# nlesc-dirac/sagecal

Measured on NVIDIA H100. Metric: baseline_visibilities_per_sec_predict_jacobian, higher is better.
Workload: dtype f64

## Files before the change

sagecal_b200/csrc/internal.cuh:

```cuda
#pragma once
#include <cuda_runtime.h>
#include <stdint.h>
#include <stdio.h>
#include <stdlib.h>

#define DB_CHECK(call)                                                                          \
  do {                                                                                          \
    cudaError_t err__ = (call);                                                                 \
    if (err__ != cudaSuccess) {                                                                 \
      fprintf(stderr, "dirac_b200: CUDA error %s at %s:%d: %s\n", cudaGetErrorName(err__),      \
              __FILE__, __LINE__, cudaGetErrorString(err__));                                   \
      exit(1);          \
    }                                                                                           \
  } while (0)


#define TILE_P 8
#define TILE_Q 32
#define TILE_THREADS (TILE_P * TILE_Q)

struct TileDesc {
  short pb, qb;
};

// ... 86 lines not shown
}
__host__ __device__ __forceinline__ void cdot2c_acc(double2 &acc, double2 a0, double2 b0, double2 a1,
                                           double2 b1) {
  acc.x = fma(a0.x, b0.x, acc.x);
  acc.x = fma(a0.y, b0.y, acc.x);
  acc.x = fma(a1.x, b1.x, acc.x);
  acc.x = fma(a1.y, b1.y, acc.x);
  acc.y = fma(a0.y, b0.x, acc.y);
  acc.y = fma(-a0.x, b0.y, acc.y);
  acc.y = fma(a1.y, b1.x, acc.y);
  acc.y = fma(-a1.x, b1.y, acc.y);
}
__host__ __device__ __forceinline__ void mat_ab(const double2 *a, const double2 *b, double2 *c) {
  c[0] = cdot2(a[0], b[0], a[1], b[2]);
  c[1] = cdot2(a[0], b[1], a[1], b[3]);
  c[2] = cdot2(a[2], b[0], a[3], b[2]);
  c[3] = cdot2(a[2], b[1], a[3], b[3]);
}
__host__ __device__ __forceinline__ void mat_abh(const double2 *a, const double2 *b, double2 *c) {
  c[0] = cdot2c(a[0], b[0], a[1], b[1]);
  c[1] = cdot2c(a[0], b[2], a[1], b[3]);
  c[2] = cdot2c(a[2], b[0], a[3], b[1]);
  c[3] = cdot2c(a[2], b[2], a[3], b[3]);
}
__host__ __device__ __forceinline__ void mat_abh_acc(const double2 *a, const double2 *b, double2 *c) {
  cdot2c_acc(c[0], a[0], b[0], a[1], b[1]);
  cdot2c_acc(c[1], a[0], b[2], a[1], b[3]);
  cdot2c_acc(c[2], a[2], b[0], a[3], b[1]);
  cdot2c_acc(c[3], a[2], b[2], a[3], b[3]);
}
__host__ __device__ __forceinline__ void mat_ahb(const double2 *a, const double2 *b, double2 *c) {
  c[0] = cadd(cmulcl(a[0], b[0]), cmulcl(a[2], b[2]));
  c[1] = cadd(cmulcl(a[0], b[1]), cmulcl(a[2], b[3]));
  c[2] = cadd(cmulcl(a[1], b[0]), cmulcl(a[3], b[2]));
  c[3] = cadd(cmulcl(a[1], b[1]), cmulcl(a[3], b[3]));
}

__device__ __forceinline__ double2 ld_stream(const double2 *p) {
  double2 v;
  asm volatile("ld.global.nc.L1::no_allocate.v2.f64 {%0,%1}, [%2];" : "=d"(v.x), "=d"(v.y) : "l"(p));
  return v;
}
__device__ __forceinline__ void st_stream(double2 *p, double2 v) {
  asm volatile("st.global.L1::no_allocate.v2.f64 [%0], {%1,%2};" ::"l"(p), "d"(v.x), "d"(v.y)
               : "memory");
}

__device__ __forceinline__ double warp_sum(double v) {
#pragma unroll
  for (int o = 16; o > 0; o >>= 1) v += __shfl_xor_sync(0xffffffffu, v, o);
  return v;
}

__device__ __forceinline__ void load_jones(const double *pblk, int sta, double2 *J) {
  const double2 *s = reinterpret_cast<const double2 *>(pblk + 8 * (long long)sta);
  J[0] = __ldg(s + 0);
  J[1] = __ldg(s + 1);
  J[2] = __ldg(s + 2);
  J[3] = __ldg(s + 3);
}

__device__ __forceinline__ int row_chunk(long long r, long long R, int nchunk) {
  return nchunk == 1 ? 0 : (int)(r / ((R + nchunk - 1) / nchunk));
}

struct GradArgs {
  const double2 *coh;
  const double2 *res;
  const unsigned char *flag;
  const double *pp;
  const ClusterDesc *clus;
  const int *chunk_poff;
  const TileDesc *tiles;
  double *g;
  long long R;
  int N, Nbase, tilesz, M;
  int robust;
  double nu;
  double scale;
  int tb0;
  long long w_lo, w_hi;
};

struct ClusterPassArgs {
  const double2 *coh_k;
  const double2 *in;
  const unsigned char *flag;
  const double *pblk;
  const TileDesc *tiles;
  double2 *out;
  double *jte;
  double *partials;
  double *cost;
  unsigned int *counter;
  long long R;
  int N, Nbase;
  int t_begin, t_end, tslice;
  int mode;
  int write_out;
  double beta;
  const double *pblk_old;
  int form_hidden;
  const short2 *blpq;
  double *jte_part;
  unsigned int *gcounter;
  const double2 *wt;
};

struct WeightedJtjArgs {
  const double2 *coh_k;
  const double2 *wt;
  const unsigned char *flag;
  const double *pblk;
  const TileDesc *tiles;
  double *JTJ;
  double *HP, *HQ;
  long long R;
  int N, Nbase;
  int t_begin, t_end, tslice;
};

// ... 110 lines not shown
```

sagecal_b200/csrc/kernels_line.cu:

```cuda
#include "internal.cuh"

__device__ __forceinline__ void grid_reduce_sum_l(double v, double *partials, double *out,
                                                  unsigned int *counter) {
  __shared__ double wsum[32];
  __shared__ bool is_last;
  v = warp_sum(v);
  const int lane = threadIdx.x & 31, w = threadIdx.x >> 5;
  if (lane == 0) wsum[w] = v;
  __syncthreads();
  const unsigned int nblocks = gridDim.x * gridDim.y;
  const unsigned int bid = blockIdx.x + gridDim.x * blockIdx.y;
  if (threadIdx.x == 0) {
    double s = 0.0;
    const int nw = (blockDim.x + 31) >> 5;
    for (int i = 0; i < nw; i++) s += wsum[i];
    partials[bid] = s;
    __threadfence();
    is_last = (atomicAdd(counter, 1u) == nblocks - 1);
  }
  __syncthreads();
  if (is_last) {
    double s = 0.0;
    for (unsigned int i = threadIdx.x; i < nblocks; i += blockDim.x)
      s += ((volatile double *)partials)[i];
// ... 62 lines not shown
    out[threadIdx.x] = s;
    if (threadIdx.x == 0) *counter = 0;
  }
}

__global__ void __launch_bounds__(256)
k_line_poly(const double2 *__restrict__ E0, const double2 *__restrict__ E1,
            const double2 *__restrict__ E2, long long n4, double *partials, double *out,
            unsigned int *counter) {
  double c[5] = {0.0, 0.0, 0.0, 0.0, 0.0};
  for (long long i = (long long)blockIdx.x * blockDim.x + threadIdx.x; i < n4;
       i += (long long)gridDim.x * blockDim.x) {
    const double2 e0 = E0[i], e1 = E1[i], e2 = E2[i];
    c[0] = fma(e0.x, e0.x, fma(e0.y, e0.y, c[0]));
    c[1] = fma(e0.x, e1.x, fma(e0.y, e1.y, c[1]));
    c[2] = fma(e1.x, e1.x, fma(e1.y, e1.y, c[2]));
    c[2] = fma(-2.0 * e0.x, e2.x, fma(-2.0 * e0.y, e2.y, c[2]));
    c[3] = fma(e1.x, e2.x, fma(e1.y, e2.y, c[3]));
    c[4] = fma(e2.x, e2.x, fma(e2.y, e2.y, c[4]));
  }
  poly_grid_reduce(c, partials, out, counter);
}

__global__ void __launch_bounds__(256)
k_line_poly_finish(const double *__restrict__ part, unsigned nparts, double *partials, double *out,
                   unsigned int *counter) {
  double c[5] = {0.0, 0.0, 0.0, 0.0, 0.0};
  for (unsigned i = blockIdx.x * blockDim.x + threadIdx.x; i < nparts; i += gridDim.x * blockDim.x)
#pragma unroll
    for (int j = 0; j < 5; j++) c[j] += part[(size_t)j * nparts + i];
  poly_grid_reduce(c, partials, out, counter);
}

__global__ void __launch_bounds__(256)
k_sumsq(const double2 *__restrict__ v, long long n4, double *partials, double *out,
        unsigned int *counter) {
  double s = 0.0;
  for (long long i = (long long)blockIdx.x * blockDim.x + threadIdx.x; i < n4;
       i += (long long)gridDim.x * blockDim.x) {
    const double2 e = v[i];
    s = fma(e.x, e.x, s);
    s = fma(e.y, e.y, s);
  }
  grid_reduce_sum_l(s, partials, out, counter);
}

__global__ void __launch_bounds__(256)
k_line_residual(const double2 *__restrict__ E0, const double2 *__restrict__ E1,
                const double2 *__restrict__ E2, double2 *__restrict__ res, long long n4,
                double alpha) {
  const double a2 = alpha * alpha;
  for (long long i = (long long)blockIdx.x * blockDim.x + threadIdx.x; i < n4;
       i += (long long)gridDim.x * blockDim.x) {
    const double2 e0 = E0[i], e1 = E1[i], e2 = E2[i];
    res[i] = make_double2((e0.x - alpha * e1.x) - a2 * e2.x, (e0.y - alpha * e1.y) - a2 * e2.y);
  }
}

__global__ void __launch_bounds__(256)
k_residual_cost(const double2 *__restrict__ x, const double2 *__restrict__ pm,
                double2 *__restrict__ out, long long n4, int out_mode, int cost_mode, double inv_nu,
                double *partials, double *cost, unsigned int *counter) {
  double s = 0.0;
  for (long long i = (long long)blockIdx.x * blockDim.x + threadIdx.x; i < n4;
       i += (long long)gridDim.x * blockDim.x) {
    const double2 xv = x[i], m = pm[i];
    const double2 e = make_double2(xv.x - m.x, xv.y - m.y);
    if (out_mode == 1) out[i] = e;
    if (out_mode == 2) out[i] = m;
    if (cost_mode == 1) {
      s = fma(e.x, e.x, s);
      s = fma(e.y, e.y, s);
    } else if (cost_mode == 2) {
      s += log(1.0 + e.x * e.x * inv_nu);
      s += log(1.0 + e.y * e.y * inv_nu);
    }
  }
  if (cost_mode) grid_reduce_sum_l(s, partials, cost, counter);
}

__global__ void __launch_bounds__(256)
k_axpby(const double2 *__restrict__ x, double2 *__restrict__ y, long long n4, double a, double b) {
  for (long long i = (long long)blockIdx.x * blockDim.x + threadIdx.x; i < n4;
       i += (long long)gridDim.x * blockDim.x) {
    const double2 xv = x[i], yv = y[i];
    y[i] = make_double2(a * xv.x + b * yv.x, a * xv.y + b * yv.y);
  }
}

__global__ void __launch_bounds__(256)
k_cluster_rowmap(const double2 *__restrict__ coh_k, const double2 *__restrict__ in,
                 const double2 *in2, double2 *out,
                 const unsigned char *__restrict__ flag, const double *__restrict__ pp,
                 const int *__restrict__ chunk_poff, int nchunk, const short2 *__restrict__ blpq,
                 long long R, int Nbase, int sign, double beta) {
  for (long long r = (long long)blockIdx.x * blockDim.x + threadIdx.x; r < R;
       r += (long long)gridDim.x * blockDim.x) {
    const short2 pq = blpq[r % Nbase];
    const int off = chunk_poff[row_chunk(r, R, nchunk)];
    double2 Jp[4], Jq[4], C[4], A[4], m[4];
    load_jones(pp + off, pq.x, Jp);
    load_jones(pp + off, pq.y, Jq);
#pragma unroll
    for (int c = 0; c < 4; c++) C[c] = coh_k[(long long)c * R + r];
    mat_ab(Jp, C, A);
    mat_abh(A, Jq, m);
    const bool fl = flag[r] != 0;
#pragma unroll
// ... 63 lines not shown
```

sagecal_b200/csrc/kernels_stream.cu:

```cuda
#include "internal.cuh"
#include "tma.cuh"

#define XP_ROWS 8
__global__ void k_coh_to_planar(const double2 *__restrict__ src, double2 *__restrict__ dst,
                                long long r0, int nr, int M, long long R) {
  __shared__ double2 tile[4][XP_ROWS][33];
  const int kx = blockIdx.x * 32 + threadIdx.x;
  const int ry = blockIdx.y * XP_ROWS + threadIdx.y;
  if (kx < M && ry < nr) {
    const double2 *s = src + ((long long)ry * M + kx) * 4;
#pragma unroll
    for (int c = 0; c < 4; c++) tile[c][threadIdx.y][threadIdx.x] = s[c];
  }
  __syncthreads();
  const int tid = threadIdx.y * 32 + threadIdx.x;
  const int rr = tid % XP_ROWS, kk = tid / XP_ROWS;
  const int k = blockIdx.x * 32 + kk;
  const int r = blockIdx.y * XP_ROWS + rr;
  if (k < M && r < nr) {
#pragma unroll
    for (int c = 0; c < 4; c++) dst[((long long)k * 4 + c) * R + r0 + r] = tile[c][rr][kk];
  }
}

// ... 92 lines not shown
template <int TB, int NST, bool WIN, bool BAND = false>
__device__ __forceinline__ void grad_tma_split_body(GradArgs a) {
  if (BAND) {
    a.coh += (long long)blockIdx.z * a.M * 4 * a.R;
    a.res += (long long)blockIdx.z * 4 * a.R;
  }
  extern __shared__ __align__(128) unsigned char smem_raw[];
  constexpr int STAGE_ELEMS = TB * 4 * 32;
  double (*sq)[8][TILE_Q] = reinterpret_cast<double (*)[8][TILE_Q]>(smem_raw);
  double2 *ring = reinterpret_cast<double2 *>(smem_raw + sizeof(double) * 2 * TILE_P * 8 * TILE_Q);
  unsigned long long *bars =
      reinterpret_cast<unsigned long long *>(ring + (size_t)TILE_P * NST * STAGE_ELEMS);
  const TileDesc td = a.tiles[blockIdx.x];
  const int h = threadIdx.x >> 8, w = (threadIdx.x >> 5) & 7, lane = threadIdx.x & 31;
  const int p = td.pb * TILE_P + w;
  const int q0 = td.qb * TILE_Q;
  const int q = q0 + lane;
  const bool valid = (q > p) && (q < a.N);
  const int t0 = (WIN ? a.tb0 + (int)blockIdx.y : (int)blockIdx.y) * TB;
  const int nrows = min(TB, a.tilesz - t0);
  const int qs = max(q0, p + 1);
  const int nv = max(0, min(q0 + TILE_Q, a.N) - qs);
  const long long b0 = nv > 0 ? baseline_index(p, qs, a.N) : 0;
  const int el = q - qs;
  const long long b = valid ? b0 + el : 0;
  double2 *my_stage = ring + (size_t)w * NST * STAGE_ELEMS;
  unsigned long long *my_bar = bars + w * NST;
  if (h == 0 && lane == 0) {
#pragma unroll
    for (int s = 0; s < NST; s++) mbar_init(&my_bar[s], 1);
    mbar_fence_init();
  }
  __syncthreads();
  auto issue = [&](int k, int s) {
    const unsigned row_bytes = (unsigned)nv * 16u;
    mbar_expect_tx(&my_bar[s], (unsigned)nrows * 4u * row_bytes);
    const double2 *ck = a.coh + (long long)k * 4 * a.R + (long long)t0 * a.Nbase + b0;
    double2 *dst = my_stage + (size_t)s * STAGE_ELEMS;
    for (int i = 0; i < nrows; i++)
#pragma unroll
      for (int c = 0; c < 4; c++)
        bulk_g2s(dst + (i * 4 + c) * 32, ck + (long long)c * a.R + (long long)i * a.Nbase, row_bytes,
                 &my_bar[s]);
  };
  const bool producer = (h == 0 && lane == 0 && nv > 0);
  if (producer) {
#pragma unroll
    for (int s = 0; s < NST - 1; s++)
      if (s < a.M) issue(s, s);
  }

  double2 Rm[TB][2];
  bool use[TB];
#pragma unroll
  for (int i = 0; i < TB; i++) {
    const int t = t0 + i;
    const long long row = (long long)(t < a.tilesz ? t : a.tilesz - 1) * a.Nbase + b;
    use[i] = valid && (t < a.tilesz) && (a.flag[row] == 0);
    if (WIN) use[i] = use[i] && row >= a.w_lo && row < a.w_hi;
#pragma unroll
    for (int j = 0; j < 2; j++) {
      double2 e = make_double2(0.0, 0.0);
      if (use[i]) {
        e = ld_stream(a.res + (long long)(2 * h + j) * a.R + row);
        if (a.robust) {
          e.x = e.x / (a.nu + e.x * e.x);
          e.y = e.y / (a.nu + e.y * e.y);
        }
      }
      Rm[i][j] = e;
    }
  }
  for (int k = 0; k < a.M; k++) {
    const int s = k % NST;
    if (producer && k + NST - 1 < a.M) issue(k + NST - 1, (k + NST - 1) % NST);
    const ClusterDesc cd = a.clus[k];
    const int tpc = (a.tilesz + cd.nchunk - 1) / cd.nchunk;
    if (nv > 0) mbar_wait(&my_bar[s], (unsigned)((k / NST) & 1));
    const double2 *st = my_stage + (size_t)s * STAGE_ELEMS;
    int i0 = 0;
    while (i0 < TB) {
      int chunk = 0, i1 = TB;
      double2 W[8];
#pragma unroll
      for (int z = 0; z < 8; z++) W[z] = make_double2(0.0, 0.0);
      if (cd.nchunk == 1) {
#pragma unroll
        for (int i = 0; i < TB; i++) {
          if (use[i]) {
            double2 C[4];
#pragma unroll
            for (int c = 0; c < 4; c++) C[c] = lds_v2(st + (i * 4 + c) * 32 + el);
#pragma unroll
            for (int j = 0; j < 2; j++)
#pragma unroll
              for (int lm = 0; lm < 4; lm++) cfmac(W[j * 4 + lm], Rm[i][j], C[lm]);
          }
        }
      } else {
        chunk = (t0 + i0 < a.tilesz ? t0 + i0 : a.tilesz - 1) / tpc;
        i1 = i0;
#pragma unroll
        for (int i = 0; i < TB; i++) {
          if (i >= i0 && i == i1) {
            const int t = t0 + i;
            const int ch = (t < a.tilesz ? t : a.tilesz - 1) / tpc;
            if (ch == chunk) {
              i1 = i + 1;
              if (use[i]) {
                double2 C[4];
#pragma unroll
                for (int c = 0; c < 4; c++) C[c] = lds_v2(st + (i * 4 + c) * 32 + el);
#pragma unroll
                for (int j = 0; j < 2; j++)
#pragma unroll
                  for (int lm = 0; lm < 4; lm++) cfmac(W[j * 4 + lm], Rm[i][j], C[lm]);
              }
// ... 506 lines not shown
      for (int i = tid; i < n8; i += 512) {
        double sacc = 0.0;
        for (unsigned c = 0; c < gridDim.y; c++) sacc += __ldcg(grp + (size_t)c * n8 + i);
        if (sacc != 0.0) atomicAdd(a.jte + i, sacc);
      }
      if (tid == 0) a.gcounter[blockIdx.x] = 0;
    }
  }
  grid_reduce_sum(cost, a.partials, a.cost, a.counter);
}


__global__ void __launch_bounds__(TILE_THREADS)
k_coh_gram(GramArgs a) {
  const TileDesc td = a.tiles[blockIdx.x];
  const int w = threadIdx.x >> 5, lane = threadIdx.x & 31;
  const int p = td.pb * TILE_P + w;
  const int q = td.qb * TILE_Q + lane;
  if (!((q > p) && (q < a.N))) return;
  const long long b = baseline_index(p, q, a.N);
  const double2 *ck = a.coh + (long long)(a.k0 + blockIdx.y) * 4 * a.R;
  double d[4] = {0.0, 0.0, 0.0, 0.0};
  double2 o[6];
#pragma unroll
  for (int z = 0; z < 6; z++) o[z] = make_double2(0.0, 0.0);
#pragma unroll 4
  for (int t = a.t_begin; t < a.t_end; t += a.t_step) {
    const long long row = (long long)t * a.Nbase + b;
    double2 C[4];
#pragma unroll
    for (int c = 0; c < 4; c++) C[c] = ld_stream(ck + (long long)c * a.R + row);
    if (a.flag[row] == 0) {
#pragma unroll
      for (int c = 0; c < 4; c++) {
        d[c] = fma(C[c].x, C[c].x, d[c]);
        d[c] = fma(C[c].y, C[c].y, d[c]);
      }
      cfmacl(o[0], C[0], C[1]);
      cfmacl(o[1], C[0], C[2]);
      cfmacl(o[2], C[0], C[3]);
      cfmacl(o[3], C[1], C[2]);
      cfmacl(o[4], C[1], C[3]);
      cfmacl(o[5], C[2], C[3]);
    }
  }
  double2 *Tb = reinterpret_cast<double2 *>(a.T + ((long long)blockIdx.y * a.Nbase + b) * 16);
  Tb[0] = make_double2(d[0], d[1]);
  Tb[1] = make_double2(d[2], d[3]);
#pragma unroll
  for (int z = 0; z < 6; z++) Tb[2 + z] = o[z];
}

void db_launch_grad_tma(const GradArgs *a, int ntile, cudaStream_t st) {
  constexpr int TB = 4, NST = 2;
  const size_t smem = sizeof(double) * 2 * TILE_P * 8 * TILE_Q +
                      (size_t)TILE_P * NST * TB * 4 * 32 * sizeof(double2) + TILE_P * NST * 8;
  static bool configured = false;
  if (!configured) {
    DB_CHECK(cudaFuncSetAttribute(k_grad_tma_split<TB, NST>,
                                  cudaFuncAttributeMaxDynamicSharedMemorySize, (int)smem));
    configured = true;
  }
  dim3 grid(ntile, (a->tilesz + TB - 1) / TB);
  k_grad_tma_split<TB, NST><<<grid, 2 * TILE_THREADS, smem, st>>>(*a);
}

void db_launch_grad_band_tma(const GradArgs *a, int ntile, int nchan, cudaStream_t st) {
  constexpr int TB = 4, NST = 2;
  const size_t smem = sizeof(double) * 2 * TILE_P * 8 * TILE_Q +
                      (size_t)TILE_P * NST * TB * 4 * 32 * sizeof(double2) + TILE_P * NST * 8;
  static bool configured = false;
  if (!configured) {
    DB_CHECK(cudaFuncSetAttribute(k_grad_tma_band<TB, NST>,
                                  cudaFuncAttributeMaxDynamicSharedMemorySize, (int)smem));
    configured = true;
  }
  dim3 grid(ntile, (a->tilesz + TB - 1) / TB, nchan);
  k_grad_tma_band<TB, NST><<<grid, 2 * TILE_THREADS, smem, st>>>(*a);
}

void db_launch_grad_window_tma(const GradArgs *a, int ntile, long long r_lo, long long r_hi,
                               cudaStream_t st) {
  constexpr int TB = 4, NST = 2;
  if (r_hi <= r_lo) return;
  const size_t smem = sizeof(double) * 2 * TILE_P * 8 * TILE_Q +
                      (size_t)TILE_P * NST * TB * 4 * 32 * sizeof(double2) + TILE_P * NST * 8;
  static bool configured = false;
  if (!configured) {
    DB_CHECK(cudaFuncSetAttribute(k_grad_tma_window<TB, NST>,
                                  cudaFuncAttributeMaxDynamicSharedMemorySize, (int)smem));
    configured = true;
  }
  const int t_lo = (int)(r_lo / a->Nbase), t_hi = (int)((r_hi + a->Nbase - 1) / a->Nbase);
  const int tb_lo = t_lo / TB, tb_hi = (t_hi + TB - 1) / TB;
  GradArgs b = *a;
  b.tb0 = tb_lo;
  b.w_lo = r_lo;
  b.w_hi = r_hi;
  dim3 grid(ntile, tb_hi - tb_lo);
  k_grad_tma_window<TB, NST><<<grid, 2 * TILE_THREADS, smem, st>>>(b);
}

static bool cluster_pass_lin_fits(int N, int Nbase) {
  return (size_t)5 * 8 * 256 * sizeof(double2) + sizeof(double) * ((8 * N + 1) & ~1) + 40 <=
             (size_t)200 * 1024 && (Nbase + 255) / 256 <= 1024;
}

// ... 79 lines not shown
```

sagecal_b200/csrc/lbfgs.cu:

```cuda
#include <float.h>
#include <math.h>
#include <string.h>
#include <vector>

#include "problem.h"

extern "C" {
int db_lbfgs_direction_max_pairs(void);
void db_launch_lbfgs_direction(double *pk, const double *gk, const double *s, const double *y,
                               const double *rho, int m, int npairs, int next, cudaStream_t st);
void db_launch_lbfgs_nrm2(const double *g, int m, double *out, cudaStream_t st);
void db_launch_lbfgs_step(const double *xk, const double *pk, const double *gk, double *xk1,
                          double *sk, double *yk, int m, double alpha, cudaStream_t st);
void db_launch_lbfgs_update(const double *gk, const double *sk, double *yk, const double *xk1,
                            double *xk, int m, double *rho_slot, double *out, cudaStream_t st);
void db_launch_line_eval(const double2 *E0, const double2 *E1, const double2 *E2, long long n4,
                         double alpha, int mode, double inv_nu, double *partials, double *out,
                         unsigned int *counter, cudaStream_t st);
void db_launch_line_residual(const double2 *E0, const double2 *E1, const double2 *E2, double2 *res,
                             long long n4, double alpha, cudaStream_t st);
void db_launch_line_poly(const double2 *E0, const double2 *E1, const double2 *E2, long long n4,
                         double *partials, double *out, unsigned int *counter, cudaStream_t st);
}

// ... 66 lines not shown
    }
    db_prof_end(d.stream);
    DB_CHECK(cudaEventRecord(ev_done, cs));
    DB_CHECK(cudaStreamWaitEvent(d.stream, ev_done, 0));
    db_launch_axpby(d.x, pr->E0, 4 * d.R, 1.0, -1.0, d.stream);
    db_count_launch(1);
  } else {
    db_prof_begin(7, (double)d.R * (64.0 * d.M + 65.0 + 192.0), d.stream);
    const unsigned nparts = db_launch_line_setup_tma(&s, d.stream);
    db_prof_end(d.stream);
    db_count_launch(1);
    if (fold_poly) {
      db_launch_line_poly_finish(pr->poly_part, nparts, pr->partials, d.scal + 16, d.counters,
                                 d.stream);
      db_count_launch(1);
    }
    if (pr->world > 1) {
      db_allreduce(pr, pr->E0, 3 * 8 * d.R);
      db_launch_axpby(d.x, pr->E0, 4 * d.R, 1.0, -1.0, d.stream);
      db_count_launch(1);
    }
  }
  if (want_poly) {
    if (!fold_poly) {
      db_launch_line_poly(pr->E0, pr->E1, pr->E2, 4 * d.R, pr->partials, d.scal + 16, d.counters,
                          d.stream);
      db_count_launch(1);
    }
    DB_CHECK(cudaMemcpyAsync(d.h_scal + 16, d.scal + 16, 5 * sizeof(double), cudaMemcpyDeviceToHost,
                             d.stream));
    db_stream_sync(d.stream);
    for (int j = 0; j < 5; j++) c->poly[j] = d.h_scal[16 + j];
  }
}

static double line_cost(LbfgsCtx *c, double alpha) {
  dirac_b200_problem *pr = c->pr;
  DevProblem &d = pr->d;
  if (!c->robust && !db_opt(DB_OPT_LINE_DIRECT)) {
    c->ncost++;
    const double *q = c->poly;
    return q[0] + alpha * (q[1] + alpha * (q[2] + alpha * (q[3] + alpha * q[4])));
  }
  db_launch_line_eval(pr->E0, pr->E1, pr->E2, 4 * d.R, alpha, c->robust ? 2 : 1,
                      c->robust ? 1.0 / c->nu : 0.0, pr->partials, d.scal, d.counters, d.stream);
  db_count_launch(1);
  c->ncost++;
  return db_read_scalar(pr, 0);
}

enum { RES_PREDICT, RES_LINE, RES_HELD };
static void grad_eval(LbfgsCtx *c, const double *p, double *g, int res_src, double alpha) {
  dirac_b200_problem *pr = c->pr;
  DevProblem &d = pr->d;
  if (res_src == RES_LINE) {
    db_launch_line_residual(pr->E0, pr->E1, pr->E2, pr->res, 4 * d.R, alpha, d.stream);
    db_count_launch(1);
  } else if (res_src == RES_PREDICT) {
    db_predict_dev(pr, p, pr->res, 1, 0, 0.0, 0);
  }
  db_grad_dev(pr, p, g, c->robust, c->nu);
  c->ngrad++;
}

static double cubic_interp(LbfgsCtx *c, double a, double b, double *xa, double step) {
  double f0, f1, f0d, f1d, p01, p02, z0, fz0, aa, cc;
  *xa = a;
  f0 = line_cost(c, *xa);
  *xa += step;
  p01 = line_cost(c, *xa);
  *xa += -2.0 * step;
  p02 = line_cost(c, *xa);
  f0d = (p01 - p02) / (2.0 * step);
  *xa += -a + step + b;
  f1 = line_cost(c, *xa);
  *xa += step;
  p01 = line_cost(c, *xa);
  *xa += -2.0 * step;
  p02 = line_cost(c, *xa);
  f1d = (p01 - p02) / (2.0 * step);

  aa = 3.0 * (f0 - f1) / (b - a) + (f1d - f0d);
  p01 = aa * aa - f0d * f1d;
  if (p01 > 0.0) {
    cc = sqrt(p01);
    z0 = b - (f1d + cc - aa) * (b - a) / (f1d - f0d + 2.0 * cc);
    aa = (a > b) ? a : b;
    cc = (a < b) ? a : b;
    if (z0 > aa || z0 < cc) {
      fz0 = f0 + f1;
    } else {
      *xa += -b + step + a + z0 * (b - a);
      fz0 = line_cost(c, *xa);
    }
    if (f0 < f1 && f0 < fz0) return a;
    if (f1 < fz0) return b;
    return z0;
  }
  return (f0 < f1) ? a : b;
}

static double linesearch_zoom(LbfgsCtx *c, double a, double b, double *xa, double phi_0,
                              double gphi_0, double sigma, double rho, double t1, double t2,
                              double t3, double step) {
  double alphaj = 0.0, phi_j, phi_aj, gphi_j, p01, p02, aj = a, bj = b, alphak = 1.0;
  int ci = 0, found_step = 0;
  (void)t1;
  while (ci < 10) {
    p01 = aj + t2 * (bj - aj);
    p02 = bj - t3 * (bj - aj);
    alphaj = cubic_interp(c, p01, p02, xa, step);
    *xa = alphaj;
    phi_j = line_cost(c, *xa);
    *xa += -alphaj + aj;
// ... 81 lines not shown
    ci++;
  }
  return alphak;
}

struct LbfgsTrace {
  double *alphak;
  long long *ncost;
  int *slot;
  double *gnorm;
  double *iterates;
  int niter;
};

static int lbfgs_run(dirac_b200_problem *pr, double *p, int m, int itmax, int M, int robust,
                      double nu, bool res_held, LbfgsTrace *tr) {
  DevProblem &d = pr->d;
  LbfgsCtx ctx;
  ctx.pr = pr;
  ctx.robust = robust;
  ctx.nu = nu;
  ctx.m = m;
  ctx.ncost = ctx.ngrad = 0;
  if (tr) tr->niter = 0;
  if (M < 1) M = 1;
  if (M > db_lbfgs_direction_max_pairs()) {
    fprintf(stderr, "dirac_b200: LBFGS memory size %d exceeds the %d pairs the two-loop recursion "
                    "can hold; the LBFGS stage is skipped\n", M, db_lbfgs_direction_max_pairs());
    return 0;
  }
  double *ws = (double *)db_malloc(sizeof(double) * ((size_t)m * (4 + 2 * (size_t)M) + M + 8));
  double *xk = ws, *xk1 = xk + m, *gk = xk1 + m, *pk = gk + m, *s = pk + m,
         *y = s + (size_t)m * M, *rho = y + (size_t)m * M;
  double *nrm_dev = d.scal + 24;
  double step, alphak;
  int ck, ci, cm;
  DB_CHECK(cudaMemcpyAsync(xk, p, sizeof(double) * m, cudaMemcpyHostToDevice, d.stream));
  grad_eval(&ctx, xk, gk, res_held ? RES_HELD : RES_PREDICT, 0.0);
  db_launch_lbfgs_nrm2(gk, m, nrm_dev, d.stream);
  db_count_launch(1);
  double gradnrm = sqrt(db_read_scalar(pr, 24));
  const double STOP = 1e-17;
  if (gradnrm < STOP) {
    ck = itmax;
    step = 0.0;
  } else {
    ck = 0;
    double t = 1e-3 / gradnrm;
    if (t > 1e-6) t = 1e-6;
    step = (t > 1e-9) ? t : 1e-9;
  }
  cm = 0;
  ci = 0;
  while (ck < itmax && isnormal(gradnrm) && gradnrm > STOP) {
    const long long ncost0 = ctx.ncost;
    db_launch_lbfgs_direction(pk, gk, s, y, rho, m, ck < M ? ck : M, ci, d.stream);
    db_count_launch(1);
    line_setup(&ctx, xk, pk);
    alphak = linesearch(&ctx, 10.0, 0.1, 0.01, 9, 0.1, 0.5, step);
    if (!isnormal(alphak) || fabs(alphak) < 1e-12) break;
    double *sk = s + (size_t)cm;
    double *yk = y + (size_t)cm;
    db_launch_lbfgs_step(xk, pk, gk, xk1, sk, yk, m, alphak, d.stream);
    grad_eval(&ctx, xk1, gk, RES_LINE, alphak);
    db_launch_lbfgs_update(gk, sk, yk, xk1, xk, m, rho + ci, nrm_dev, d.stream);
    db_count_launch(2);
    gradnrm = sqrt(db_read_scalar(pr, 24));
    if (tr) {
      tr->alphak[ck] = alphak;
      tr->ncost[ck] = ctx.ncost - ncost0;
      tr->slot[ck] = ci;
      tr->gnorm[ck] = gradnrm;
      DB_CHECK(cudaMemcpy(tr->iterates + (size_t)m * ck, xk, sizeof(double) * m,
                          cudaMemcpyDeviceToHost));
      tr->niter = ck + 1;
    }
    ck++;
    if (cm < (M - 1) * m) {
      cm += m;
      ci++;
    } else {
      cm = ci = 0;
    }
  }
  DB_CHECK(cudaMemcpyAsync(p, xk, sizeof(double) * m, cudaMemcpyDeviceToHost, d.stream));
  db_stream_sync(d.stream);
  db_free(ws);
  return (int)ctx.ngrad - 1;
}

int db_lbfgs_fit(dirac_b200_problem *pr, double *p, int m, int itmax, int M, int robust,
                 double nu, bool res_held) {
  return lbfgs_run(pr, p, m, itmax, M, robust, nu, res_held, nullptr);
}

extern "C" void dirac_b200_line_model(dirac_b200_problem *pr, const double *xk, const double *pk,
                                      int nalpha, const double *alphas, double nu,
                                      double alpha_res, double *E, double *poly, double *costs,
                                      double *res, int *shape) {
  DevProblem &d = pr->d;
  LbfgsCtx c;
  c.pr = pr; c.robust = 0; c.nu = nu; c.m = (int)d.npar; c.ncost = c.ngrad = 0;
  double *dx = (double *)db_malloc(sizeof(double) * 2 * d.npar);
  double *dp = dx + d.npar;
  DB_CHECK(cudaMemcpyAsync(dx, xk, sizeof(double) * d.npar, cudaMemcpyHostToDevice, d.stream));
  DB_CHECK(cudaMemcpyAsync(dp, pk, sizeof(double) * d.npar, cudaMemcpyHostToDevice, d.stream));
  db_line_setup_shape_reset();
  line_setup(&c, dx, dp);
  db_line_setup_shape(shape);
  for (int j = 0; j < 5; j++) poly[j] = c.poly[j];
  for (int i = 0; i < nalpha; i++)
    for (int mode = 1; mode <= 2; mode++) {
      db_launch_line_eval(pr->E0, pr->E1, pr->E2, 4 * d.R, alphas[i], mode,
                          mode == 2 ? 1.0 / nu : 0.0, pr->partials, d.scal, d.counters, d.stream);
      costs[2 * i + mode - 1] = db_read_scalar(pr, 0);
    }
  db_download_vis(pr, pr->E0, E);
  db_download_vis(pr, pr->E1, E + 8 * d.R);
  db_download_vis(pr, pr->E2, E + 16 * d.R);
  db_launch_line_residual(pr->E0, pr->E1, pr->E2, pr->res, 4 * d.R, alpha_res, d.stream);
  db_download_vis(pr, pr->res, res);
  DB_CHECK(cudaGetLastError());
  db_free(dx);
}

extern "C" void dirac_b200_line_poly(dirac_b200_problem *pr, double *poly) {
  DevProblem &d = pr->d;
  db_launch_line_poly(pr->E0, pr->E1, pr->E2, 4 * d.R, pr->partials, d.scal + 16, d.counters,
                      d.stream);
  DB_CHECK(cudaMemcpyAsync(d.h_scal + 16, d.scal + 16, 5 * sizeof(double), cudaMemcpyDeviceToHost,
                           d.stream));
  db_stream_sync(d.stream);
  DB_CHECK(cudaGetLastError());
  for (int j = 0; j < 5; j++) poly[j] = d.h_scal[16 + j];
}

extern "C" void dirac_b200_residual(dirac_b200_problem *pr, double *out) {
  db_download_vis(pr, pr->res, out);
  DB_CHECK(cudaGetLastError());
}

extern "C" int dirac_b200_lbfgs_trace(dirac_b200_problem *pr, double *p, int itmax, int M, int robust,
                                      double nu, double *alphak, long long *ncost, int *slot,
                                      double *gnorm, double *iterates) {
  if ((M < 1 ? 1 : M) > db_lbfgs_direction_max_pairs()) return -1;
  LbfgsTrace tr;
  tr.alphak = alphak; tr.ncost = ncost; tr.slot = slot; tr.gnorm = gnorm; tr.iterates = iterates;
  lbfgs_run(pr, p, (int)pr->d.npar, itmax, M, robust, nu, false, &tr);
  return tr.niter;
}

extern "C" int dirac_b200_lbfgs_direction(int m, int Mmem, int npairs, int next, const double *g,
                                          const double *s, const double *y, const double *rho,
                                          double *pk) {
  if (m < 1 || Mmem < 1 || npairs < 0 || npairs > Mmem || next < 0 || next >= Mmem ||
      npairs > db_lbfgs_direction_max_pairs())
    return -1;
  const size_t nv = (size_t)m * (2 + 2 * (size_t)Mmem) + Mmem;
  double *w = (double *)db_malloc(sizeof(double) * nv);
  double *dg = w, *dpk = dg + m, *ds = dpk + m, *dy = ds + (size_t)m * Mmem,
         *drho = dy + (size_t)m * Mmem;
  DB_CHECK(cudaMemcpy(dg, g, sizeof(double) * m, cudaMemcpyHostToDevice));
  DB_CHECK(cudaMemcpy(ds, s, sizeof(double) * m * Mmem, cudaMemcpyHostToDevice));
  DB_CHECK(cudaMemcpy(dy, y, sizeof(double) * m * Mmem, cudaMemcpyHostToDevice));
  DB_CHECK(cudaMemcpy(drho, rho, sizeof(double) * Mmem, cudaMemcpyHostToDevice));
  db_launch_lbfgs_direction(dpk, dg, ds, dy, drho, m, npairs, next, 0);
  DB_CHECK(cudaGetLastError());
  DB_CHECK(cudaMemcpy(pk, dpk, sizeof(double) * m, cudaMemcpyDeviceToHost));
  db_free(w);
  return 0;
}

extern "C" int dirac_b200_lbfgs_step_update(int m, double alpha, const double *xk, const double *pk,
                                            const double *gk_old, const double *gk_new, int Mmem,
                                            int ci, const double *rho_in, double *xk1, double *sk,
                                            double *yk, double *rho, double *gg, double *xk_out) {
  if (m < 1 || Mmem < 1 || ci < 0 || ci >= Mmem) return -1;
  const size_t nv = (size_t)m * 7 + Mmem + 1;
// ... 33 lines not shown
```

sagecal_b200/csrc/problem.cu:

```cuda
#include <string.h>
#include <thread>
#include <vector>

#include "../../include/dirac_b200.h"
#include "internal.cuh"
#include "problem.h"

static unsigned long long g_launches = 0;
static unsigned long long g_sky_uploads = 0, g_coh_host_bytes = 0;
void db_count_sky_upload() { g_sky_uploads++; }
void db_count_coh_host_bytes(size_t bytes) { g_coh_host_bytes += bytes; }
extern "C" void dirac_b200_transfer_stats(unsigned long long *sky_uploads,
                                          unsigned long long *coh_host_bytes, int reset) {
  if (sky_uploads) *sky_uploads = g_sky_uploads;
  if (coh_host_bytes) *coh_host_bytes = g_coh_host_bytes;
  if (reset) g_sky_uploads = g_coh_host_bytes = 0;
}
void db_count_launch(int n) { g_launches += (unsigned long long)n; }
extern "C" unsigned long long dirac_b200_launch_count(void) { return g_launches; }

struct ProfRec { cudaEvent_t a, b; int kind; double bytes; };
static std::vector<ProfRec> g_prof;
static std::vector<cudaEvent_t> g_evpool;
static int g_prof_on = 0;
// ... 412 lines not shown
  for (long long r0 = 0; r0 < R; r0 += rows_per) {
    int nr = (int)((R - r0 < rows_per) ? (R - r0) : rows_per);
    db_launch_coh_from_planar(coh, stage, r0, nr, M, R, st);
    db_count_launch(1);
    DB_CHECK(cudaMemcpyAsync(x + (size_t)r0 * M * 8, stage, (size_t)nr * M * 64,
                             cudaMemcpyDeviceToHost, st));
  }
  db_stream_sync(st);
  db_count_coh_host_bytes((size_t)R * M * 64);
  db_free(stage);
}

extern "C" void dirac_b200_get_coherencies(dirac_b200_problem *pr, double *coh) {
  db_download_coh(pr->d.coh, coh, pr->d.M, pr->d.R, pr->d.stream);
}

void db_predict_dev(dirac_b200_problem *pr, const double *pp_dev, double2 *out, int out_mode,
                    int cost_mode, double nu, int slot) {
  DevProblem &d = pr->d;
  StreamAllArgs a;
  memset(&a, 0, sizeof(a));
  a.coh = d.coh; a.x = d.x; a.flag = d.flag; a.pp = pp_dev; a.clus = d.clus;
  a.chunk_poff = d.chunk_poff; a.blpq = d.blpq; a.out = out; a.partials = pr->partials;
  a.cost = d.scal + slot; a.counter = d.counters; a.R = d.R; a.N = d.N; a.Nbase = d.Nbase;
  a.tilesz = d.tilesz; a.M = d.M; a.out_mode = out_mode; a.cost_mode = cost_mode;
  a.inv_nu = (nu > 0.0) ? 1.0 / nu : 0.0;
  if (pr->world > 1) {
    if (!pr->pm) pr->pm = dev_alloc<double2>((size_t)4 * d.R);
    a.out = pr->pm; a.out_mode = 2; a.cost_mode = 0;
    db_prof_begin(0, (double)d.R * (64.0 * d.M + 65.0 + 64.0), d.stream);
    db_launch_predict_tma(&a, d.stream);
    db_prof_end(d.stream);
    db_allreduce(pr, pr->pm, 8 * d.R);
    db_launch_residual_cost(d.x, pr->pm, out, 4 * d.R, out ? out_mode : 0, cost_mode, a.inv_nu,
                            pr->partials, d.scal + slot, d.counters, d.stream);
    db_count_launch(2);
    return;
  }
  db_prof_begin(0, (double)d.R * (64.0 * d.M + 65.0 + (out_mode ? 64.0 : 0.0)), d.stream);
  db_launch_predict_tma(&a, d.stream);
  db_prof_end(d.stream);
  db_count_launch(1);
}

double db_read_scalar(dirac_b200_problem *pr, int slot) {
  DevProblem &d = pr->d;
  DB_CHECK(cudaMemcpyAsync(d.h_scal + slot, d.scal + slot, sizeof(double), cudaMemcpyDeviceToHost,
                           d.stream));
  db_stream_sync(d.stream);
  return d.h_scal[slot];
}

void db_grad_dev(dirac_b200_problem *pr, const double *pp_dev, double *g_dev, int robust,
                 double nu) {
  DevProblem &d = pr->d;
  DB_CHECK(cudaMemsetAsync(g_dev, 0, sizeof(double) * d.npar, d.stream));
  GradArgs a;
  a.coh = d.coh; a.res = pr->res; a.flag = d.flag; a.pp = pp_dev; a.clus = d.clus;
  a.chunk_poff = d.chunk_poff; a.tiles = d.tiles; a.g = g_dev; a.R = d.R; a.N = d.N;
  a.Nbase = d.Nbase; a.tilesz = d.tilesz; a.M = d.M; a.robust = robust; a.nu = nu;
  a.scale = robust ? -2.0 : 2.0;
  db_prof_begin(1, (double)d.R * (64.0 * d.M + 65.0) + 64.0 * d.N * d.Mt, d.stream);
  db_launch_grad_tma(&a, d.ntile, d.stream);
  db_prof_end(d.stream);
  db_count_launch(1);
  db_allreduce(pr, g_dev, d.npar);
}

double db_cost_window_dev(dirac_b200_problem *pr, const double *pp_dev, double2 *out, double nu,
                          long long r_lo, long long r_hi) {
  DevProblem &d = pr->d;
  if (r_lo < 0) r_lo = 0;
  if (r_hi > d.R) r_hi = d.R;
  if (r_hi <= r_lo) return 0.0;
  const long long t_lo = r_lo / d.Nbase, t_hi = (r_hi + d.Nbase - 1) / d.Nbase;
  const long long r0 = t_lo * d.Nbase, len = r_hi - r_lo;
  StreamAllArgs a;
  memset(&a, 0, sizeof(a));
  a.coh = d.coh + r0; a.x = d.x + r0; a.flag = d.flag + r0; a.pp = pp_dev; a.clus = d.clus;
  a.chunk_poff = d.chunk_poff; a.blpq = d.blpq; a.partials = pr->partials;
  a.cost = d.scal; a.counter = d.counters; a.R = d.R; a.N = d.N; a.Nbase = d.Nbase;
  a.tilesz = (int)(t_hi - t_lo); a.M = d.M; a.row0 = r0;
  a.w_lo = r_lo - r0; a.w_hi = r_hi - r0;
  a.inv_nu = (nu > 0.0) ? 1.0 / nu : 0.0;
  const double bytes = (double)len * (64.0 * d.M + 65.0 + (out ? 64.0 : 0.0));
  if (pr->world <= 1) {
    a.out = out ? out + r0 : nullptr;
    a.out_mode = out ? 1 : 0;
    a.cost_mode = 2;
    db_prof_begin(0, bytes, d.stream);
    db_launch_cost_window_tma(&a, d.stream);
    db_prof_end(d.stream);
    db_count_launch(1);
    return db_read_scalar(pr, 0);
  }
  if (!pr->pm) pr->pm = dev_alloc<double2>((size_t)4 * d.R);
  a.out = pr->pm + r0; a.out_mode = 2; a.cost_mode = 0;
  db_prof_begin(0, bytes, d.stream);
  db_launch_cost_window_tma(&a, d.stream);
  db_prof_end(d.stream);
  for (int c = 0; c < 4; c++) db_allreduce(pr, pr->pm + (long long)c * d.R + r_lo, 2 * len);
  for (int c = 0; c < 4; c++) {
    const long long off = (long long)c * d.R + r_lo;
    db_launch_residual_cost(d.x + off, pr->pm + off, out ? out + off : nullptr, len, out ? 1 : 0, 2,
                            a.inv_nu, pr->partials, d.scal + 32 + c, d.counters, d.stream);
  }
  db_count_launch(5);
  DB_CHECK(cudaMemcpyAsync(d.h_scal + 32, d.scal + 32, 4 * sizeof(double), cudaMemcpyDeviceToHost,
                           d.stream));
  db_stream_sync(d.stream);
  return ((d.h_scal[32] + d.h_scal[33]) + d.h_scal[34]) + d.h_scal[35];
}

void db_grad_window_dev(dirac_b200_problem *pr, const double *pp_dev, double *g_dev, double nu,
                        long long r_lo, long long r_hi) {
// ... 67 lines not shown
```

sagecal_b200/csrc/problem.h:

```cpp
#pragma once
#include <cusolverDn.h>
#include <cublas_v2.h>

#include <vector>

#include "../../include/dirac_b200.h"
#include "internal.cuh"

struct BigChol;
BigChol *db_bigchol_create(int n, int nbk, bool inv_panel, bool lookahead);
enum { BC_BLOCK = 256 };
static const bool BC_INV_PANEL = true, BC_LOOKAHEAD = true;
void db_bigchol_destroy(BigChol *bc);
void db_bigchol_bind_batch(BigChol *bc, double *A0, long long stride, int maxb);
void db_bigchol_factor_batch(BigChol *bc, int nb, int *info, int info_step, cudaStream_t st);

struct LMWork {
  bool ready;
  int n8;
  double *T;
  unsigned char *T_valid;
  double *Tsub;
  double *JTJ0, *JTJ;
  double *JTe, *JTe_new;
// ... 60 lines not shown
  double *poly_part;
  struct RtrWork *rtr;
};

void db_stream_sync(cudaStream_t st);
void db_event_sync(cudaEvent_t ev);
void db_flag_wait(const volatile unsigned long long *flag, unsigned long long epoch,
                  cudaStream_t st);
void *db_malloc(size_t bytes);
void db_free(void *p);
size_t db_cached_bytes();
void require_gpu();

class DeviceScope {
 public:
  DeviceScope();
  explicit DeviceScope(cudaStream_t borrowed);
  ~DeviceScope();
  DeviceScope(const DeviceScope &) = delete;
  DeviceScope &operator=(const DeviceScope &) = delete;
  template <class T> T *alloc(size_t n) {
    void *p = nullptr;
    DB_CHECK(cudaMalloc(&p, sizeof(T) * n));
    bufs_.push_back(p);
    return (T *)p;
  }
  template <class T> T *upload(const T *h, size_t n) {
    T *d = alloc<T>(n ? n : 1);
    if (n) DB_CHECK(cudaMemcpyAsync(d, h, sizeof(T) * n, cudaMemcpyHostToDevice, st));
    return d;
  }
  template <class T> T *upload(const std::vector<T> &h) { return upload(h.data(), h.size()); }
  void sync();
  const cudaStream_t st;

 private:
  const bool own_;
  std::vector<void *> bufs_;
};

void db_download_coh(const double2 *coh, double *x, int M, long long R, cudaStream_t st);
void db_count_launch(int n);
void db_prof_begin(int kind, double bytes, cudaStream_t st);
void db_prof_end(cudaStream_t st);
int db_prof_open(int kind, double bytes, cudaStream_t st);
void db_prof_close(int rec, cudaStream_t st);
cudaStream_t db_new_stream(int *owned);
void db_upload_vis(dirac_b200_problem *pr, const double *h, double2 *dst);
void db_download_vis(dirac_b200_problem *pr, const double2 *src, double *h);
void db_predict_dev(dirac_b200_problem *pr, const double *pp_dev, double2 *out, int out_mode,
                    int cost_mode, double nu, int slot);
double db_read_scalar(dirac_b200_problem *pr, int slot);
void db_grad_dev(dirac_b200_problem *pr, const double *pp_dev, double *g_dev, int robust,
                 double nu);
double db_cost_window_dev(dirac_b200_problem *pr, const double *pp_dev, double2 *out, double nu,
                          long long r_lo, long long r_hi);
void db_grad_window_dev(dirac_b200_problem *pr, const double *pp_dev, double *g_dev, double nu,
                        long long r_lo, long long r_hi);
int db_bfgsfit_dev(dirac_b200_problem *pr, double *pp, int max_lbfgs, int lbfgs_m, int solver_mode,
                   double mean_nu, double *res_0, double *res_1, bool keep_residual);
void db_count_sky_upload();
void db_count_coh_host_bytes(size_t bytes);
void db_lm_init(dirac_b200_problem *pr);
void db_prefactor_sweep(dirac_b200_problem *pr, double tau);
void db_allreduce(dirac_b200_problem *pr, void *dev, long long count);
void db_allreduce_world(dirac_b200_problem *pr, void *dev, long long count);
int db_nccl_world();
void db_allreduce_stream(dirac_b200_allreduce_fn fn, void *user, void *dev, long long count,
                         cudaStream_t st);
int db_manifold_projectback(double *Y, int n, int Mt, int Nf, int Niter, const int *cr,
                            cudaStream_t st);void db_lm_set_aug(const double *y_dev, const double *bz_dev, const double *y_host,
                   const double *bz_host, double rho);
int db_overlap_available(const dirac_b200_problem *pr);
cudaStream_t db_comm_stream();
void db_allreduce_segments(dirac_b200_problem *pr, double **ptr, const long long *count, int nseg,
                           cudaStream_t st);
extern "C" {
void db_launch_residual_cost(const double2 *x, const double2 *pm, double2 *out, long long n4,
                             int out_mode, int cost_mode, double inv_nu, double *partials,
                             double *cost, unsigned int *counter, cudaStream_t st);
void db_launch_sumsq(const double2 *v, long long n4, double *partials, double *out,
                     unsigned int *counter, cudaStream_t st);
void db_launch_axpby(const double2 *x, double2 *y, long long n4, double a, double b,
                     cudaStream_t st);
void db_launch_cluster_rowmap(const double2 *coh_k, const double2 *in, const double2 *in2,
                              double2 *out, const unsigned char *flag, const double *pp,
                              const int *chunk_poff, int nchunk, const short2 *blpq, long long R,
                              int Nbase, int sign, double beta, cudaStream_t st);
}

struct BandView {
  const double2 *coh, *x;
  const unsigned char *flag;
  int nc;
};
struct BandDev {
  int N, Nbase, tilesz, M, Mt, maxnc, ntile;
  long long R, npar;
  ClusterDesc *clus;
  int *chunk_poff;
  TileDesc *tiles;
  short2 *blpq;
  double *pp, *g, *partials, *scal, *h_scal;
  unsigned int *counters;
  double2 *res;
  cudaStream_t st;
};
// ... 14 lines not shown
```

Before: 7.613 billion.

## Fuse line-search residual into gradient kernel and defer residual materialisation

The gradient kernel can now build the residual on the fly from E0, E1, E2 and alpha, so the separate line-residual kernel no longer runs before every gradient evaluation in L-BFGS. The residual buffer is written only once after the loop ends, using the last accepted step. The gradient tile also grows from 4 to 6 timeslots per thread, which uses more registers and shared memory. This removes a full read/write pass over the residual at each gradient, but each gradient now reads three streams instead of one. The predict/Jacobian metric may not touch this path at all.

```diff
diff --git a/profiles/lbfgs_c4.py b/profiles/lbfgs_c4.py
--- /dev/null
+++ b/profiles/lbfgs_c4.py
@@ -0,0 +1,96 @@
+import argparse
+import json
+import os
+import subprocess
+import sys
+
+import numpy as np
+
+ROOT = os.path.dirname(os.path.dirname(os.path.abspath(__file__)))
+sys.path.insert(0, ROOT)
+
+from sagecal_b200 import lib as blib
+from sagecal_b200 import synth
+from sagecal_b200.dirac_api import SkyModel, make_barr
+
+GRAD, LINE_SETUP = 1, 7
+
+
+def card():
+    import torch
+    name = torch.cuda.get_device_name(0)
+    try:
+        q = subprocess.run(["nvidia-smi", "--query-gpu=power.limit,clocks.max.sm",
+                            "--format=csv,noheader", "-i", "0"], capture_output=True, text=True,
+                           timeout=30).stdout.strip()
+    except (OSError, subprocess.TimeoutExpired):
+        q = "power limit not read"
+    return "%s, %s" % (name, q)
+
+
+def main():
+    ap = argparse.ArgumentParser()
+    ap.add_argument("--lib", default=blib.LIB_PATH)
+    ap.add_argument("--iters", type=int, default=10, help="max_lbfgs of the timed stage")
+    ap.add_argument("--reps", type=int, default=3, help="timed stages (after one warm-up)")
+    args = ap.parse_args()
+    import torch
+    api = blib.DiracB200(os.path.abspath(args.lib))
+    c = synth.CONFIGS["C4"]
+    pr = synth.make_problem(with_data=False, N=c["N"], M=32, tilesz=c["tilesz"], radius=c["radius"],
+                            seed=c["seed"], kmean=c["kmean"])
+    barr = make_barr(pr.sta1, pr.sta2, pr.flag)
+    sky = SkyModel(pr.clusters, pr.N)
+    R = pr.Nbase1
+    x = np.zeros(8 * R)
+    dp = blib.DeviceProblem(api, pr.N, pr.Nbase, pr.tilesz, barr, sky, None, x)
+    dp.precalculate(pr.u, pr.v, pr.w, pr.freq0, pr.fdelta)
+    model = np.zeros(8 * R)
+    api.lib.dirac_b200_predict(dp.h, blib.dptr(pr.jones_true), blib.dptr(model), 2, 0, 0.0)
+    rng = np.random.default_rng(c["seed"] + 17)
+    sigma = 1e-2 * np.median(np.abs(model[:: max(1, len(model) // 4000000)]))
+    x = model + rng.normal(0, sigma, model.shape)
+    del model
+    x.reshape(R, 8)[pr.flag == 1] = 0.0
+    dp.set_data(x)
+
+    def stage(max_lbfgs):
+        pp = pr.pp0.copy()
+        e0, e1 = torch.cuda.Event(enable_timing=True), torch.cuda.Event(enable_timing=True)
+        n0 = api.kernel_count(LINE_SETUP)
+        e0.record()
+        res = dp.sagefit(pp, None, max_emiter=0, max_iter=2, max_lbfgs=max_lbfgs, lbfgs_m=7)
+        e1.record()
+        torch.cuda.synchronize()
+        return e0.elapsed_time(e1), api.kernel_count(LINE_SETUP) - n0, res
+
+    stage(args.iters)
+    stage(0)
+    walls, bases, nlines = [], [], set()
+    for _ in range(args.reps):
+        ms, nl, res = stage(args.iters)
+        walls.append(ms)
+        nlines.add(nl)
+        bases.append(stage(0)[0])
+    api.profile_enable(True)
+    stage(args.iters)
+    prof = {k: api.profile_read(k) for k in (GRAD, LINE_SETUP)}
+    api.profile_enable(False)
+    nl = max(nlines)
+    out = {"card": card(), "lib": os.path.relpath(os.path.abspath(args.lib), ROOT),
+           "shape": "N=%d, Nbase=%d, M=32, tilesz=%d, rows=%d" % (pr.N, pr.Nbase, pr.tilesz, R),
+           "line_setups_per_stage": sorted(nlines), "res_1": res[3]}
+    for k, name in ((LINE_SETUP, "line_model_pass"), (GRAD, "gradient_pass")):
+        n, ms, by = prof[k]
+        out[name] = {"launches": n, "ms_per_launch": ms / n, "GB_per_launch": by / n / 1e9,
+                     "GB_s": by / (ms * 1e-3) / 1e9}
+    it = [(w - b) / nl for w, b in zip(walls, bases)]
+    out["lbfgs_iteration_ms"] = {"mean": float(np.mean(it)), "min": float(np.min(it)),
+                                 "max": float(np.max(it))}
+    out["stage_ms"] = walls
+    print(json.dumps(out))
+    dp.close()
+
+
+if __name__ == "__main__":
+    main()
diff --git a/sagecal_b200/csrc/internal.cuh b/sagecal_b200/csrc/internal.cuh
--- a/sagecal_b200/csrc/internal.cuh
+++ b/sagecal_b200/csrc/internal.cuh
@@ -162,6 +162,11 @@
   return v;
 }
 
+__device__ __forceinline__ double2 line_residual(double2 e0, double2 e1, double2 e2, double alpha,
+                                                double a2) {
+  return make_double2((e0.x - alpha * e1.x) - a2 * e2.x, (e0.y - alpha * e1.y) - a2 * e2.y);
+}
+
 __device__ __forceinline__ void load_jones(const double *pblk, int sta, double2 *J) {
   const double2 *s = reinterpret_cast<const double2 *>(pblk + 8 * (long long)sta);
   J[0] = __ldg(s + 0);
@@ -177,6 +182,8 @@
 struct GradArgs {
   const double2 *coh;
   const double2 *res;
+  const double2 *E1, *E2;
+  double alpha;
   const unsigned char *flag;
   const double *pp;
   const ClusterDesc *clus;
diff --git a/sagecal_b200/csrc/kernels_line.cu b/sagecal_b200/csrc/kernels_line.cu
--- a/sagecal_b200/csrc/kernels_line.cu
+++ b/sagecal_b200/csrc/kernels_line.cu
@@ -138,8 +138,7 @@
   const double a2 = alpha * alpha;
   for (long long i = (long long)blockIdx.x * blockDim.x + threadIdx.x; i < n4;
        i += (long long)gridDim.x * blockDim.x) {
-    const double2 e0 = E0[i], e1 = E1[i], e2 = E2[i];
-    res[i] = make_double2((e0.x - alpha * e1.x) - a2 * e2.x, (e0.y - alpha * e1.y) - a2 * e2.y);
+    res[i] = line_residual(E0[i], E1[i], E2[i], alpha, a2);
   }
 }
 
diff --git a/sagecal_b200/csrc/kernels_stream.cu b/sagecal_b200/csrc/kernels_stream.cu
--- a/sagecal_b200/csrc/kernels_stream.cu
+++ b/sagecal_b200/csrc/kernels_stream.cu
@@ -168,6 +168,7 @@
 
   double2 Rm[TB][2];
   bool use[TB];
+  const double a2 = a.alpha * a.alpha;
 #pragma unroll
   for (int i = 0; i < TB; i++) {
     const int t = t0 + i;
@@ -178,7 +179,9 @@
     for (int j = 0; j < 2; j++) {
       double2 e = make_double2(0.0, 0.0);
       if (use[i]) {
-        e = ld_stream(a.res + (long long)(2 * h + j) * a.R + row);
+        const long long ix = (long long)(2 * h + j) * a.R + row;
+        e = ld_stream(a.res + ix);
+        if (a.E1) e = line_residual(e, ld_stream(a.E1 + ix), ld_stream(a.E2 + ix), a.alpha, a2);
         if (a.robust) {
           e.x = e.x / (a.nu + e.x * e.x);
           e.y = e.y / (a.nu + e.y * e.y);
@@ -791,7 +794,7 @@
 }
 
 void db_launch_grad_tma(const GradArgs *a, int ntile, cudaStream_t st) {
-  constexpr int TB = 4, NST = 2;
+  constexpr int TB = 6, NST = 2;
   const size_t smem = sizeof(double) * 2 * TILE_P * 8 * TILE_Q +
                       (size_t)TILE_P * NST * TB * 4 * 32 * sizeof(double2) + TILE_P * NST * 8;
   static bool configured = false;
diff --git a/sagecal_b200/csrc/lbfgs.cu b/sagecal_b200/csrc/lbfgs.cu
--- a/sagecal_b200/csrc/lbfgs.cu
+++ b/sagecal_b200/csrc/lbfgs.cu
@@ -142,14 +142,8 @@
 enum { RES_PREDICT, RES_LINE, RES_HELD };
 static void grad_eval(LbfgsCtx *c, const double *p, double *g, int res_src, double alpha) {
   dirac_b200_problem *pr = c->pr;
-  DevProblem &d = pr->d;
-  if (res_src == RES_LINE) {
-    db_launch_line_residual(pr->E0, pr->E1, pr->E2, pr->res, 4 * d.R, alpha, d.stream);
-    db_count_launch(1);
-  } else if (res_src == RES_PREDICT) {
-    db_predict_dev(pr, p, pr->res, 1, 0, 0.0, 0);
-  }
-  db_grad_dev(pr, p, g, c->robust, c->nu);
+  if (res_src == RES_PREDICT) db_predict_dev(pr, p, pr->res, 1, 0, 0.0, 0);
+  db_grad_dev(pr, p, g, c->robust, c->nu, res_src == RES_LINE, alpha);
   c->ngrad++;
 }
 
@@ -337,13 +331,18 @@
   }
   cm = 0;
   ci = 0;
+  bool have_line = false;
+  double a_res = 0.0;
   while (ck < itmax && isnormal(gradnrm) && gradnrm > STOP) {
     const long long ncost0 = ctx.ncost;
     db_launch_lbfgs_direction(pk, gk, s, y, rho, m, ck < M ? ck : M, ci, d.stream);
     db_count_launch(1);
     line_setup(&ctx, xk, pk);
+    have_line = true;
+    a_res = 0.0;
     alphak = linesearch(&ctx, 10.0, 0.1, 0.01, 9, 0.1, 0.5, step);
     if (!isnormal(alphak) || fabs(alphak) < 1e-12) break;
+    a_res = alphak;
     double *sk = s + (size_t)cm;
     double *yk = y + (size_t)cm;
     db_launch_lbfgs_step(xk, pk, gk, xk1, sk, yk, m, alphak, d.stream);
@@ -368,6 +367,10 @@
       cm = ci = 0;
     }
   }
+  if (have_line) {
+    db_launch_line_residual(pr->E0, pr->E1, pr->E2, pr->res, 4 * d.R, a_res, d.stream);
+    db_count_launch(1);
+  }
   DB_CHECK(cudaMemcpyAsync(p, xk, sizeof(double) * m, cudaMemcpyDeviceToHost, d.stream));
   db_stream_sync(d.stream);
   db_free(ws);
@@ -409,6 +412,22 @@
   db_free(dx);
 }
 
+extern "C" void dirac_b200_line_grad(dirac_b200_problem *pr, const double *p, double alpha,
+                                     int robust, double nu, double *g_line, double *g_res) {
+  DevProblem &d = pr->d;
+  double *w = (double *)db_malloc(sizeof(double) * 2 * d.npar);
+  double *dp = w, *dg = w + d.npar;
+  DB_CHECK(cudaMemcpyAsync(dp, p, sizeof(double) * d.npar, cudaMemcpyHostToDevice, d.stream));
+  db_grad_dev(pr, dp, dg, robust, nu, true, alpha);
+  DB_CHECK(cudaMemcpyAsync(g_line, dg, sizeof(double) * d.npar, cudaMemcpyDeviceToHost, d.stream));
+  db_launch_line_residual(pr->E0, pr->E1, pr->E2, pr->res, 4 * d.R, alpha, d.stream);
+  db_grad_dev(pr, dp, dg, robust, nu);
+  DB_CHECK(cudaMemcpyAsync(g_res, dg, sizeof(double) * d.npar, cudaMemcpyDeviceToHost, d.stream));
+  db_stream_sync(d.stream);
+  DB_CHECK(cudaGetLastError());
+  db_free(w);
+}
+
 extern "C" void dirac_b200_line_poly(dirac_b200_problem *pr, double *poly) {
   DevProblem &d = pr->d;
   db_launch_line_poly(pr->E0, pr->E1, pr->E2, 4 * d.R, pr->partials, d.scal + 16, d.counters,
diff --git a/sagecal_b200/csrc/problem.cu b/sagecal_b200/csrc/problem.cu
--- a/sagecal_b200/csrc/problem.cu
+++ b/sagecal_b200/csrc/problem.cu
@@ -488,15 +488,23 @@
 }
 
 void db_grad_dev(dirac_b200_problem *pr, const double *pp_dev, double *g_dev, int robust,
-                 double nu) {
+                 double nu, bool from_line, double alpha) {
   DevProblem &d = pr->d;
   DB_CHECK(cudaMemsetAsync(g_dev, 0, sizeof(double) * d.npar, d.stream));
   GradArgs a;
-  a.coh = d.coh; a.res = pr->res; a.flag = d.flag; a.pp = pp_dev; a.clus = d.clus;
+  memset(&a, 0, sizeof(a));
+  a.coh = d.coh; a.flag = d.flag; a.pp = pp_dev; a.clus = d.clus;
+  a.res = from_line ? pr->E0 : pr->res;
+  if (from_line) {
+    a.E1 = pr->E1;
+    a.E2 = pr->E2;
+    a.alpha = alpha;
+  }
   a.chunk_poff = d.chunk_poff; a.tiles = d.tiles; a.g = g_dev; a.R = d.R; a.N = d.N;
   a.Nbase = d.Nbase; a.tilesz = d.tilesz; a.M = d.M; a.robust = robust; a.nu = nu;
   a.scale = robust ? -2.0 : 2.0;
-  db_prof_begin(1, (double)d.R * (64.0 * d.M + 65.0) + 64.0 * d.N * d.Mt, d.stream);
+  db_prof_begin(1, (double)d.R * (64.0 * d.M + 65.0 + (from_line ? 128.0 : 0.0)) + 64.0 * d.N * d.Mt,
+                d.stream);
   db_launch_grad_tma(&a, d.ntile, d.stream);
   db_prof_end(d.stream);
   db_count_launch(1);
diff --git a/sagecal_b200/csrc/problem.h b/sagecal_b200/csrc/problem.h
--- a/sagecal_b200/csrc/problem.h
+++ b/sagecal_b200/csrc/problem.h
@@ -136,7 +136,7 @@
                     int cost_mode, double nu, int slot);
 double db_read_scalar(dirac_b200_problem *pr, int slot);
 void db_grad_dev(dirac_b200_problem *pr, const double *pp_dev, double *g_dev, int robust,
-                 double nu);
+                 double nu, bool from_line = false, double alpha = 0.0);
 double db_cost_window_dev(dirac_b200_problem *pr, const double *pp_dev, double2 *out, double nu,
                           long long r_lo, long long r_hi);
 void db_grad_window_dev(dirac_b200_problem *pr, const double *pp_dev, double *g_dev, double nu,
```

Measured after the change: 7.812 billion (median of 6 runs). +2.6%, better.
